# HybridRobotics/ilqr-iterative-tasks

Measured on AMD Instinct MI355X. Metric: batched iLQR iterations/s (n=6,m=2,N=20), higher is better.
Workload: dtype f64

## Files before the change

### ilqr_iterative_tasks_amd/csrc/i2lqr_abi.hip

```cpp
#include <hip/hip_runtime.h>
#include <dlfcn.h>
#include <rccl/rccl.h>

#include <atomic>
#include <cmath>
#include <cstdarg>
#include <cstdio>
#include <cstdlib>
#include <cstring>
#include <mutex>
#include <new>
#include <unordered_set>

#include "../../include/i2lqr.h"
#include "i2lqr_devcfg.hpp"
#include "i2lqr_geometry.hpp"
#include "i2lqr_group.h"
#include "i2lqr_lane.hpp"
#include "i2lqr_select.hpp"
#include "i2lqr_wave.hpp"

#include "i2lqr_lane12.h"

#define I2LQR_DRY_RUN_LANE 1
// ... 203 lines not shown
#ifdef I2LQR_DEBUG
  if (rc != I2LQR_OK) return rc;
  unsigned long long* w = i2lqr::debug_trap_word();
  if (!w) return rc;
  hipStreamCaptureStatus cap = hipStreamCaptureStatusNone;
  if (hipStreamIsCapturing((hipStream_t)stream, &cap) == hipSuccess &&
      cap != hipStreamCaptureStatusNone)
    return rc;
  if (hipStreamSynchronize((hipStream_t)stream) != hipSuccess)
    return fail(I2LQR_ERR_LAUNCH, "debug build: the stream reported an error");
  unsigned long long rec = 0;
  if (hipMemcpy(&rec, w, sizeof(rec), hipMemcpyDeviceToHost) != hipSuccess)
    return fail(I2LQR_ERR_LAUNCH, "debug build: could not read the violation record");
  if (rec) {
    (void)hipMemset(w, 0, sizeof(rec));
    static const char* const names[] = {"?", "wave-kernel LDS slice", "eight-lane LDS slice",
                                        "sixteen-lane LDS slice", "quad12 HBM workspace slot",
                                        "lane kernel row of X", "lane kernel row of U / k",
                                        "lane kernel row of K", "lane kernel LDS word",
                                        "compaction row / problem index"};
    const int tag = (int)((rec >> 56) & 0x7f);
    return fail(I2LQR_ERR_LAUNCH, "debug build: index check failed: %s, index %lld, limit %lld",
                names[tag < 10 ? tag : 0], (long long)((rec >> 28) & 0xfffffff),
                (long long)(rec & 0xfffffff));
  }
#else
  (void)stream;
#endif
  return rc;
}
}

struct i2lqr_handle {
  i2lqr_config cfg;
  int lanes;
  size_t lds_bytes;
  int device;
  void* ws;
  int64_t ws_bytes;
  int64_t compact_min_batch;
  int opt_defer, opt_reroll, opt_lds_steps, opt_merge, opt_ckpt, opt_stagger;
  int wave_tail;
  int opt_pair;
  int opt_two_x;
  int opt_chunk_step;
  int opt_fuse;
  int opt_final_round;
  int opt_first_chunk;
  int opt_fstep;
  int opt_group;
  int opt_spec;
  int opt_group_ws;
  int opt_group_overlap;
  int opt_group_fixed;
  struct Epilogue {
    const int32_t* qfun;
    int outer_iter, max_relax_iter;
    void* cost_it;
    void* part;
    int64_t* best_idx;
    void* best_cost;
    bool fused;
  };
  static constexpr unsigned kTickets = 16;
  unsigned* ticket;
  std::atomic<unsigned> ticket_next;
  hipEvent_t ev_ready, ev_side_done;
  bool side_pending;
  DeviceGeometry geo;
};

namespace {
thread_local i2lqr_handle::Epilogue* t_epi = nullptr;
}

namespace {

enum FusedKernel { K_WAVE, K_GROUP, K_GROUP16, K_GROUP_WS, K_SPEC, K_SPEC16, K_QUAD, K_INVALID };
constexpr int64_t kAutoGroupBatch = 1024;
constexpr int64_t kAutoSpecBatch = 12288;

FusedKernel select_fused(const i2lqr_handle* h, int64_t B, bool early_exit, const char** why) {
  static const char* none = "";
  if (!why) why = &none;
  const bool m2 = h->cfg.m == 2 && h->cfg.n + h->cfg.m <= 8;
  const bool q16 = h->cfg.n + h->cfg.m == 16;
  if (m2) {
    const bool can = group_supported(h->cfg);
    if (h->opt_group == 8 && !can) {
      *why = "\"group_lanes\" = 8 needs a bicycle plant with Q = R = 0 and a horizon whose eight "
             "problem slices fit a CU's LDS";
      return K_INVALID;
    }
    const bool can_spec16 = group_spec_supported(h->cfg, 16), can_spec8 = group_spec_supported(h->cfg, 8);
    const bool spec16 = h->opt_group == 16 || (h->opt_group < 0 && can_spec16);
    const bool can_spec = spec16 ? can_spec16 : can_spec8;
    if (h->opt_spec == 1 && !can_spec) {
      *why = "\"speculate\" = 1 needs the eight- / sixteen-lane kernel and a horizon whose speculative "
             "buffers fit a CU's LDS";
      return K_INVALID;
    }
    if (can_spec && h->opt_group != 64 &&
        (h->opt_spec == 1 ||
         (h->opt_spec < 0 && h->opt_group < 0 && early_exit && B <= h->geo.scaled(kAutoSpecBatch))))
      return spec16 ? K_SPEC16 : K_SPEC;
    const bool can16 = group16_supported(h->cfg);
// ... 84 lines not shown
           {(const void*)k_iterate<T, Sys, LANES, false>, (const void*)k_iterate<T, Sys, LANES, true>,
            (const void*)k_backward<T, Sys, LANES, false>, (const void*)k_backward<T, Sys, LANES, true>,
            (const void*)k_forward<T, Sys, LANES, false>, (const void*)k_forward<T, Sys, LANES, true>,
            (const void*)k_rollout<T, Sys, LANES, false>, (const void*)k_rollout<T, Sys, LANES, true>})
        HIP_TRY(hipFuncSetAttribute(kernel, hipFuncAttributeMaxDynamicSharedMemorySize,
                                    (int)h->lds_bytes));
    return I2LQR_OK;
  }

  static int iterate(i2lqr_handle* h, int64_t B, int n_iters, int early_exit, void* X, void* U,
                     const void* x_term, void* lamb, const void* obs, void* cost, void* K, void* k,
                     int32_t* iters, int32_t* status, hipStream_t s) {
    const Cfg c = make_dev_cfg<T, n, m>(h->cfg);
    IterArgs<T> a = iter_args<T>(B, n_iters, early_exit, X, U, x_term, lamb, obs, cost, K, k, iters,
                                 status);
#ifdef I2LQR_STAMPS
    a.dbg = (unsigned long long*)h->ws;
#endif
    const char* why = "";
    const FusedKernel fk = select_fused(h, B, early_exit != 0, &why);
    if (t_epi && (fk == K_GROUP || fk == K_GROUP16 || fk == K_GROUP_WS)) {
      a.qfun = t_epi->qfun;
      a.outer_iter = t_epi->outer_iter;
      a.max_relax_iter = t_epi->max_relax_iter;
      a.cost_it = (T*)t_epi->cost_it;
      if (t_epi->best_idx) {
        a.pick_part = (MinPair<T>*)t_epi->part;
        a.pick_ticket = h->ticket + h->ticket_next.fetch_add(1, std::memory_order_relaxed) %
                                        i2lqr_handle::kTickets;
        a.best_idx = t_epi->best_idx;
        a.best_cost = (T*)t_epi->best_cost;
      }
      t_epi->fused = true;
    }
    switch (fk) {
      case K_INVALID:
        return fail(I2LQR_ERR_UNSUPPORTED, "%s", why);
      case K_SPEC:
      case K_SPEC16:
        if constexpr (m == 2 && n + m <= 8) {
          HIP_TRY(group_spec_iterate<T>(h->cfg, a, s, fk == K_SPEC16 ? 16 : 8));
          return I2LQR_OK;
        }
        break;
      case K_GROUP:
        if constexpr (m == 2 && n + m <= 8) {
          HIP_TRY(group_iterate<T>(h->cfg, a, s));
          return I2LQR_OK;
        }
        break;
      case K_GROUP16:
        if constexpr (m == 2 && n + m <= 8) {
          HIP_TRY(group16_iterate<T>(h->cfg, a, s, h->opt_group_overlap != 0,
                                     h->opt_group_fixed != 0));
          return I2LQR_OK;
        }
        break;
      case K_GROUP_WS:
        if constexpr (m == 2 && n + m <= 8) {
          HIP_TRY(group_iterate_ws<T>(h->cfg, a, h->ws, s));
          return I2LQR_OK;
        }
        break;
      case K_QUAD:
        if constexpr (n + m == 16) {
          HIP_TRY(quad_iterate<T>(h->cfg, a, h->ws, s));
          return I2LQR_OK;
        }
        break;
      case K_WAVE:
        break;
    }
    const size_t lds_f = fstep_lds_bytes(h->cfg.N);
    const int64_t waves_per_cu = (grid(B) + h->geo.cus - 1) / h->geo.cus;
    const bool fstep = kHasFstep && lds_f <= h->geo.default_dyn_lds &&
                       (h->opt_fstep >= 0 ? h->opt_fstep != 0
                                          : waves_per_cu * lds_f <= h->geo.lds_per_cu - 10 * 1024);
    if constexpr (kHasFstep) {
      if (fstep) {
        with_weights(c.flags, [&](auto W) {
          hipLaunchKernelGGL((k_iterate<T, Sys, LANES, W, true>), dim3(grid(B)), dim3(64), lds_f, s, c, a);
        });
        HIP_TRY(hipGetLastError());
        return I2LQR_OK;
      }
    }
    with_weights(c.flags, [&](auto W) {
      hipLaunchKernelGGL((k_iterate<T, Sys, LANES, W>), dim3(grid(B)), dim3(64), h->lds_bytes, s, c, a);
    });
    HIP_TRY(hipGetLastError());
    return I2LQR_OK;
  }
  static int names_pair(i2lqr_handle*, int64_t, int) { return 0; }
  static int solve_chained(i2lqr_handle* h, int64_t L, int k, void* X, void* U, const void* x_term,
                           void* lamb, const void* obs, void* cost, void* K, void* kk, int32_t* iters,
                           int32_t* status, hipStream_t s) {
    if constexpr (m == 2 && n + m <= 8) {
      if (h->opt_spec == 0 || h->opt_group == 8 || h->opt_group == 64 ||
          !group_spec_chain_supported(h->cfg, L))
        return fail(I2LQR_ERR_UNSUPPORTED, "chains run on the sixteen-lane speculative kernel: a "
                    "bicycle plant with Q = R = 0, at most %lld chains, a horizon whose three-wavefront "
                    "buffers fit a CU's LDS (solve the chain steps one after the other instead)",
                    (long long)h->geo.scaled(512));
      IterArgs<T> a = iter_args<T>(L, h->cfg.max_iter, 1, X, U, x_term, lamb, obs, cost, K, kk, iters,
                                   status);
      a.chain_len = k;
      HIP_TRY(group_spec_chain<T>(h->cfg, a, s));
// ... 753 lines not shown
  }
  if (cfg->n != n || cfg->m != m)
    return fail(I2LQR_ERR_INVALID, "system %d has n=%d m=%d, config says n=%d m=%d", cfg->system_id,
                n, m, cfg->n, cfg->m);
  if (cfg->N < 1 || cfg->N > I2LQR_MAX_HORIZON)
    return fail(I2LQR_ERR_INVALID, "horizon %d outside [1, %d]", cfg->N, I2LQR_MAX_HORIZON);
  if (cfg->dtype != I2LQR_F64 && cfg->dtype != I2LQR_F32)
    return fail(I2LQR_ERR_INVALID, "unknown dtype %d", cfg->dtype);
  if (cfg->layout != I2LQR_LAYOUT_PROBLEM_MAJOR && cfg->layout != I2LQR_LAYOUT_BATCH_MINOR &&
      cfg->layout != I2LQR_LAYOUT_BATCH_TILED)
    return fail(I2LQR_ERR_INVALID, "unknown layout %d", cfg->layout);
  if (!(cfg->dt > 0) || !(cfg->lamb_factor > 1) || cfg->max_iter < 0)
    return fail(I2LQR_ERR_INVALID, "need dt > 0, lamb_factor > 1, max_iter >= 0");
  for (int a = 0; a < m; a++)
    if (!(cfg->u_max[a] > 0)) return fail(I2LQR_ERR_INVALID, "u_max[%d] must be > 0", a);
  if (cfg->layout != I2LQR_LAYOUT_PROBLEM_MAJOR) {
    for (int i = 0; i < n; i++)
      for (int j = 0; j < i; j++)
        if (cfg->Q[i * I2LQR_MAX_N + j] != cfg->Q[j * I2LQR_MAX_N + i] ||
            cfg->Qt[i * I2LQR_MAX_N + j] != cfg->Qt[j * I2LQR_MAX_N + i])
          return fail(I2LQR_ERR_UNSUPPORTED, "the batch-minor / batch-tiled layouts need "
                      "symmetric Q and Qterminal (use the problem-major layout otherwise)");
    for (int a = 0; a < m; a++)
      for (int b = 0; b < a; b++)
        if (cfg->R[a * I2LQR_MAX_M + b] != cfg->R[b * I2LQR_MAX_M + a])
          return fail(I2LQR_ERR_UNSUPPORTED, "the batch-minor / batch-tiled layouts need a "
                      "symmetric R (use the problem-major layout otherwise)");
  }
  int ndev = 0;
#ifdef I2LQR_DRY_RUN
  const bool dry_run = dry::on();
#else
  constexpr bool dry_run = false;
#endif
  if (!dry_run && (hipGetDeviceCount(&ndev) != hipSuccess || ndev <= 0))
    return fail(I2LQR_ERR_NODEVICE, "no HIP device visible (this library has no CPU path)");
  i2lqr_handle* h = new (std::nothrow) i2lqr_handle;
  if (!h) return fail(I2LQR_ERR_LAUNCH, "out of host memory");
  h->cfg = *cfg;
  h->geo = device_geometry();
  if (h->geo.wave != 64) {
    const int w = h->geo.wave;
    delete h;
    return fail(I2LQR_ERR_UNSUPPORTED, "the kernels are built for 64-lane wavefronts (gfx950), this "
                "device reports %d", w);
  }
  h->ws = nullptr;
  h->ws_bytes = 0;
  h->compact_min_batch = -1;
  h->opt_defer = h->opt_reroll = h->opt_lds_steps = h->opt_fstep = h->opt_group = -1;
  h->opt_merge = h->opt_ckpt = h->opt_spec = h->opt_stagger = h->opt_group_ws = -1;
  h->opt_group_overlap = -1;
  h->opt_group_fixed = -1;
  h->wave_tail = -1;
  h->opt_first_chunk = -1;
  h->opt_fuse = -1;
  h->opt_final_round = -1;
  h->opt_chunk_step = -1;
  h->opt_pair = -1;
  h->opt_two_x = -1;
  h->ticket = nullptr;
  h->ticket_next.store(0);
  h->ev_ready = h->ev_side_done = nullptr;
  h->side_pending = false;
  constexpr size_t kTicketBytes = i2lqr_handle::kTickets * sizeof(unsigned);
  if (dry_run) {
#ifdef I2LQR_DRY_RUN
    static unsigned fake_tickets[i2lqr_handle::kTickets];
    h->device = 0;
    h->ticket = fake_tickets;
    dry::allow(fake_tickets, sizeof(fake_tickets));
#endif
  } else if (hipGetDevice(&h->device) != hipSuccess ||
      hipMalloc((void**)&h->ticket, kTicketBytes) != hipSuccess ||
      hipMemset(h->ticket, 0, kTicketBytes) != hipSuccess) {
    if (h->ticket) (void)hipFree(h->ticket);
    delete h;
    return fail(I2LQR_ERR_LAUNCH, "could not set up the handle's device state: %s",
                hipGetErrorString(hipGetLastError()));
  }
  const int rc = dispatch(h, [&](auto L) { return L.prepare(h); });
  if (rc != I2LQR_OK) {
    (void)hipFree(h->ticket);
    delete h;
    return rc;
  }
  {
    std::lock_guard<std::mutex> lock(g_live_mu);
    live_handles().insert(h);
  }
  *out = h;
  g_err[0] = 0;
  return I2LQR_OK;
}

int64_t i2lqr_dry_run(int32_t op, void* p, int64_t n) {
#ifdef I2LQR_DRY_RUN
  switch (op) {
    case 0: return dry::on() ? 1 : 0;
    case 1: if (!dry::on()) break; dry::allow(p, (size_t)n); return 0;
    case 2: if (!dry::on()) break; dry::reset(); return 0;
    case 3: if (!dry::on()) break; return dry::report((char*)p, n);
    default: return fail(I2LQR_ERR_INVALID, "i2lqr_dry_run: unknown operation %d", op);
  }
  return fail(I2LQR_ERR_UNSUPPORTED, "dry-run launches need I2LQR_DRY_RUN=1 in the environment");
#else
// ... 93 lines not shown
  for (int a = 0; a < cfg->m; a++)
    for (int b = 0; b < cfg->m; b++)
      if (cfg->R[a * I2LQR_MAX_M + b] != cfg->R[b * I2LQR_MAX_M + a]) lane_ok = false;
  int64_t from;
  switch (cfg->system_id) {
    case I2LQR_SYS_BICYCLE4:
    case I2LQR_SYS_BICYCLE6:
      from = weights ? kLaneFromWeights
                     : (early_exit ? lane_from(*cfg).solve : lane_from(*cfg).iterate);
      break;
    case I2LQR_SYS_QUAD12: {
      const LaneFrom q = kLaneFromQuad[cfg->N <= 31 ? 0 : 1][cfg->dtype == I2LQR_F64 ? 0 : 1];
      from = weights ? kLaneFromWeights : (early_exit ? q.solve : q.iterate);
      if (cfg->dtype != I2LQR_F64 && weights) lane_ok = false;
      break;
    }
    default: return fail(I2LQR_ERR_INVALID, "unknown system_id %d", cfg->system_id);
  }
  from = device_geometry().scaled_from(from);
  if (!lane_ok || B < from) return I2LQR_LAYOUT_PROBLEM_MAJOR;
  return B % 64 == 0 ? I2LQR_LAYOUT_BATCH_TILED : I2LQR_LAYOUT_BATCH_MINOR;
}

int i2lqr_set_compaction(i2lqr_handle* h, int64_t min_batch) {
  if (!h) return fail(I2LQR_ERR_INVALID, "null handle");
  if (h->cfg.layout == I2LQR_LAYOUT_PROBLEM_MAJOR && min_batch > 0)
    return fail(I2LQR_ERR_UNSUPPORTED, "compaction applies to the batch-minor / batch-tiled layouts");
  h->compact_min_batch = min_batch < 0 ? -1 : min_batch;
  return I2LQR_OK;
}

int i2lqr_set_option(i2lqr_handle* h, const char* name, int64_t value) {
  if (!h || !name) return fail(I2LQR_ERR_INVALID, "null handle or option name");
  if (value < -1 || value > 0x7fffffff) return fail(I2LQR_ERR_INVALID, "option value out of range");
  const int v = (int)value;
  if (!strcmp(name, "defer_states")) h->opt_defer = v < 0 ? -1 : (v != 0);
  else if (!strcmp(name, "reroll_nominal")) h->opt_reroll = v < 0 ? -1 : (v != 0);
  else if (!strcmp(name, "lds_gain_steps")) h->opt_lds_steps = v;
  else if (!strcmp(name, "merge_inputs")) h->opt_merge = v < 0 ? -1 : (v != 0);
  else if (!strcmp(name, "checkpoint_states")) h->opt_ckpt = v < 0 ? -1 : (v != 0);
  else if (!strcmp(name, "stagger")) h->opt_stagger = v;
  else if (!strcmp(name, "per_step_jacobians")) h->opt_fstep = v < 0 ? -1 : (v != 0);
  else if (!strcmp(name, "wave_tail")) h->wave_tail = v < 0 ? -1 : (v > 65536 ? 65536 : v);
  else if (!strcmp(name, "first_chunk")) h->opt_first_chunk = v < 1 ? -1 : (v > 1024 ? 1024 : v);
  else if (!strcmp(name, "helper_wavefront")) h->opt_pair = v < 0 ? -1 : (v != 0);
  else if (!strcmp(name, "state_buffers")) h->opt_two_x = v < 0 ? -1 : (v != 0);
  else if (!strcmp(name, "chunk_step")) h->opt_chunk_step = v < 1 ? -1 : (v > 1024 ? 1024 : v);
  else if (!strcmp(name, "fused_compaction")) h->opt_fuse = v < 0 ? -1 : (v != 0);
  else if (!strcmp(name, "final_round")) h->opt_final_round = v < 0 ? -1 : (v > 20 ? 20 : v);
  else if (!strcmp(name, "speculate")) h->opt_spec = v < 0 ? -1 : (v != 0);
  else if (!strcmp(name, "group_workspace")) h->opt_group_ws = v < 0 ? -1 : (v != 0);
  else if (!strcmp(name, "group_overlap")) h->opt_group_overlap = v < 0 ? -1 : (v != 0);
  else if (!strcmp(name, "group_fixed_horizon")) h->opt_group_fixed = v < 0 ? -1 : (v != 0);
  else if (!strcmp(name, "debug_self_test")) {
#ifdef I2LQR_DEBUG
    unsigned long long* w = i2lqr::debug_trap_word();
    double* buf = nullptr;
    HIP_TRY(hipMalloc((void**)&buf, 8 * sizeof(double)));
    hipLaunchKernelGGL(k_debug_self_test, dim3(1), dim3(64), 0, (hipStream_t)0, buf, w);
    const int rc = debug_check(I2LQR_OK, nullptr);
    (void)hipFree(buf);
    return rc;
#else
    return fail(I2LQR_ERR_UNSUPPORTED, "\"debug_self_test\" exists in the index-checked debug build "
                "only (make -C ilqr_iterative_tasks_amd/csrc debug)");
#endif
  }
  else if (!strcmp(name, "group_lanes")) {
    if (v != -1 && v != 8 && v != 16 && v != 64)
      return fail(I2LQR_ERR_INVALID, "\"group_lanes\" is 8, 16, 64 or -1");
    h->opt_group = v;
  }
  else return fail(I2LQR_ERR_INVALID, "unknown option '%s'", name);
  return I2LQR_OK;
}

static const char* kernel_name(const i2lqr_handle* h, int64_t B, bool early_exit) {
  if (!h) return "";
  if (h->cfg.layout != I2LQR_LAYOUT_PROBLEM_MAJOR) {
    if (h->cfg.system_id == I2LQR_SYS_QUAD12) return "k_lane_iterate_rows";
    const auto pair = [&](auto L) {
      return L.names_pair(const_cast<i2lqr_handle*>(h), B, early_exit ? 1 : 0);
    };
    return dispatch(h, pair) == 1 ? "k_lane_iterate_pair" : "k_lane_iterate";
  }
  switch (select_fused(h, B, early_exit, nullptr)) {
    case K_SPEC: return "k_group_spec";
    case K_SPEC16: return "k_group_spec (sixteen lanes)";
    case K_GROUP: return "k_group_iterate";
    case K_GROUP16: return "k_group_iterate (sixteen lanes)";
    case K_GROUP_WS: return "k_group_iterate (workspace form)";
    case K_QUAD: return "k_quad_iterate";
    case K_WAVE: return "k_iterate";
    default: return "unsupported";
  }
}

const char* i2lqr_iterate_kernel(const i2lqr_handle* h, int64_t B) { return kernel_name(h, B, false); }
const char* i2lqr_solve_kernel(const i2lqr_handle* h, int64_t B) { return kernel_name(h, B, true); }

int i2lqr_set_workspace(i2lqr_handle* h, void* workspace, int64_t bytes) {
  if (!h) return fail(I2LQR_ERR_INVALID, "null handle");
  if (bytes < 0 || (bytes > 0 && !workspace) || ((uintptr_t)workspace & 15))
    return fail(I2LQR_ERR_INVALID, "workspace must be a 16-byte aligned device pointer");
  h->ws = workspace;
  h->ws_bytes = bytes;
// ... 558 lines not shown
```

### ilqr_iterative_tasks_amd/csrc/i2lqr_group.h

```cpp
#pragma once
#include <hip/hip_runtime.h>

#include "../../include/i2lqr.h"
#include "i2lqr_wave.hpp"

namespace i2lqr {

bool group_supported(const i2lqr_config& cfg);
template <class T> hipError_t group_iterate(const i2lqr_config& cfg, const IterArgs<T>& a,
                                            hipStream_t stream);

constexpr int64_t kGroup16Batch = 4096;
bool group16_supported(const i2lqr_config& cfg);
template <class T> hipError_t group16_iterate(const i2lqr_config& cfg, const IterArgs<T>& a,
                                              hipStream_t stream, bool overlap = true,
                                              bool fixed = true);
#define I2LQR_GROUP_FIXED_HORIZONS(X) X(20)
bool group16_fixed_horizon(int N);
template <class T> hipError_t group16_iterate_fixed(const i2lqr_config& cfg, const IterArgs<T>& a,
                                                    hipStream_t stream, int wavefronts);

constexpr int64_t kGroupWsBatch = 4096;
constexpr int64_t kGroupWsTop = 8192;
constexpr int64_t kGroupWsTopF32 = 7168;
inline int64_t group_ws_top(const i2lqr_config& cfg) {
  return cfg.dtype == I2LQR_F64 ? kGroupWsTop : kGroupWsTopF32;
}
int64_t group_workspace_bytes(const i2lqr_config& cfg, int64_t B);
template <class T> hipError_t group_iterate_ws(const i2lqr_config& cfg, const IterArgs<T>& a,
                                               void* ws, hipStream_t stream);

bool group_spec_supported(const i2lqr_config& cfg, int lanes);
template <class T> hipError_t group_spec_iterate(const i2lqr_config& cfg, const IterArgs<T>& a,
                                                 hipStream_t stream, int lanes);
bool group_spec_chain_supported(const i2lqr_config& cfg, int64_t chains);
template <class T> hipError_t group_spec_chain(const i2lqr_config& cfg, const IterArgs<T>& a,
                                               hipStream_t stream);
bool group_spec_tail_supported(const i2lqr_config& cfg);
template <class T> hipError_t group_spec_tail(const i2lqr_config& cfg, const IterArgs<T>& a,
                                              hipStream_t stream);

bool quad_supported(const i2lqr_config& cfg);
int64_t quad_workspace_bytes(const i2lqr_config& cfg, int64_t B);
template <class T> hipError_t quad_iterate(const i2lqr_config& cfg, const IterArgs<T>& a, void* ws,
                                           hipStream_t stream);

}
```

### ilqr_iterative_tasks_amd/csrc/i2lqr_group.hip

```cpp
#include "i2lqr_group.h"

#include "i2lqr_devcfg.hpp"
#include "i2lqr_geometry.hpp"
#include "i2lqr_group.hpp"
#include "i2lqr_dryrun.hpp"
#include "i2lqr_group_launch.hpp"

namespace i2lqr {

namespace {

template <class T, class Sys, int H, int G = kGroup>
hipError_t launch_h(const i2lqr_config& cfg, const IterArgs<T>& a, hipStream_t s) {
  const auto c = make_dev_cfg<T, Sys::n, Sys::m>(cfg);
  const size_t lds = group_lds_bytes<T, Sys, G>(cfg.N);
  if (hipError_t e = raise_lds_limit<k_group_iterate<T, Sys, H, false, G>>(lds); e != hipSuccess)
    return e;
  constexpr int PW = 64 / G;
  const unsigned grid = (unsigned)((a.B + PW - 1) / PW);
  hipLaunchKernelGGL((k_group_iterate<T, Sys, H, false, G>), dim3(grid), dim3(64 * H), lds, s, c, a,
                     (T*)nullptr);
  return hipGetLastError();
}
template <class T, class Sys>
hipError_t launch16(const i2lqr_config& cfg, const IterArgs<T>& a, hipStream_t s, bool overlap,
                    bool fixed) {
  const int64_t cus = device_geometry().cus;
  int wavefronts = 1;
#ifndef I2LQR_STAMPS
  if (overlap && (a.B + 3) / 4 <= cus) wavefronts = 3;
  else if ((a.B + 3) / 4 <= 2 * cus) wavefronts = 2;
  if (fixed && group16_fixed_horizon(cfg.N)) return group16_iterate_fixed<T>(cfg, a, s, wavefronts);
#endif
  if (wavefronts == 3) return launch_h<T, Sys, 3, 16>(cfg, a, s);
  if (wavefronts == 2) return launch_h<T, Sys, 2, 16>(cfg, a, s);
  return launch_h<T, Sys, 1, 16>(cfg, a, s);
}
template <class T, class Sys>
hipError_t launch_ws(const i2lqr_config& cfg, const IterArgs<T>& a, void* ws, hipStream_t s) {
  const auto c = make_dev_cfg<T, Sys::n, Sys::m>(cfg);
  const size_t lds = (size_t)GLayout<Sys>(cfg.N, true).wave_words() * sizeof(T);
  if (hipError_t e = raise_lds_limit<k_group_iterate<T, Sys, 1, true>>(lds); e != hipSuccess) return e;
  const unsigned grid = (unsigned)((a.B + kGroupsPerWave - 1) / kGroupsPerWave);
  hipLaunchKernelGGL((k_group_iterate<T, Sys, 1, true>), dim3(grid), dim3(64), lds, s, c, a, (T*)ws);
  return hipGetLastError();
}

template <class T, class Sys>
hipError_t launch(const i2lqr_config& cfg, const IterArgs<T>& a, hipStream_t s) {
  const int64_t cus = device_geometry().cus;
#ifndef I2LQR_STAMPS
  if ((a.B + kGroupsPerWave - 1) / kGroupsPerWave <= cus) return launch_h<T, Sys, 3>(cfg, a, s);
#endif
  return launch_h<T, Sys, 1>(cfg, a, s);
}

constexpr int kSpecWideBatch = 512;

template <class T, class Sys, int V, int G = kGroup> size_t spec_lds_bytes(int N) {
  return (size_t)GSpecLayout<Sys, V, G>(N).group_words() * sizeof(T);
}

template <class T, class Sys, int V, bool SETIO, int G>
hipError_t launch_spec_v(const i2lqr_config& cfg, const IterArgs<T>& a, hipStream_t s) {
  const auto c = make_dev_cfg<T, Sys::n, Sys::m>(cfg);
  const size_t lds = spec_lds_bytes<T, Sys, V, G>(cfg.N);
  if (hipError_t e = raise_lds_limit<k_group_spec<T, Sys, V, SETIO, G>>(lds); e != hipSuccess)
    return e;
  constexpr int PW = 64 / G;
  const int64_t problems = SETIO ? (int64_t)a.count_max : a.B;
  const unsigned grid = (unsigned)((problems + PW - 1) / PW);
  hipLaunchKernelGGL((k_group_spec<T, Sys, V, SETIO, G>), dim3(grid), dim3(64 * V), lds, s, c, a);
  return hipGetLastError();
}
template <class T, class Sys, bool SETIO, int G>
hipError_t launch_spec(const i2lqr_config& cfg, const IterArgs<T>& a, hipStream_t s) {
  const DeviceGeometry& geo = device_geometry();
  const bool wide = !SETIO && a.B <= geo.scaled(kSpecWideBatch) &&
                    spec_lds_bytes<T, Sys, 3, G>(cfg.N) <= geo.max_dyn_lds;
  if (wide) return launch_spec_v<T, Sys, 3, SETIO, G>(cfg, a, s);
  return launch_spec_v<T, Sys, 2, SETIO, G>(cfg, a, s);
}
template <class T, bool SETIO>
hipError_t launch_spec_any(const i2lqr_config& cfg, const IterArgs<T>& a, hipStream_t s, int lanes) {
  return visit_bicycle<T>(cfg, [&](auto, auto sys) {
    using Sys = decltype(sys);
// ... 19 lines not shown
  });
  return lds <= device_geometry().max_dyn_lds;
}

}

bool group_spec_supported(const i2lqr_config& cfg, int lanes) {
  if (!spec_plant_ok(cfg) || cfg.layout != I2LQR_LAYOUT_PROBLEM_MAJOR) return false;
  return lanes == 16 ? spec_lds_fits<16>(cfg) : (group_supported(cfg) && spec_lds_fits<kGroup>(cfg));
}
int group_spec_tail_lanes(const i2lqr_config& cfg) {
  if (!spec_plant_ok(cfg)) return 0;
  return spec_lds_fits<16>(cfg) ? 16 : (spec_lds_fits<kGroup>(cfg) ? kGroup : 0);
}
bool group_spec_tail_supported(const i2lqr_config& cfg) { return group_spec_tail_lanes(cfg) != 0; }

template <class T, class Sys>
hipError_t launch_spec_chain(const i2lqr_config& cfg, const IterArgs<T>& a, hipStream_t s) {
  const auto c = make_dev_cfg<T, Sys::n, Sys::m>(cfg);
  const size_t lds = spec_lds_bytes<T, Sys, 3, 16>(cfg.N);
  if (hipError_t e = raise_lds_limit<k_group_spec<T, Sys, 3, false, 16, true>>(lds); e != hipSuccess)
    return e;
  const unsigned grid = (unsigned)((a.B + 3) / 4);
  hipLaunchKernelGGL((k_group_spec<T, Sys, 3, false, 16, true>), dim3(grid), dim3(64 * 3), lds, s, c, a);
  return hipGetLastError();
}
bool group_spec_chain_supported(const i2lqr_config& cfg, int64_t chains) {
  if (!spec_plant_ok(cfg) || cfg.layout != I2LQR_LAYOUT_PROBLEM_MAJOR) return false;
  const DeviceGeometry& geo = device_geometry();
  if (chains > geo.scaled(kSpecWideBatch)) return false;
  const size_t lds = visit_bicycle(cfg, [&](auto t, auto sys) {
    return spec_lds_bytes<decltype(t), decltype(sys), 3, 16>(cfg.N);
  });
  return lds <= geo.max_dyn_lds;
}
template <class T>
hipError_t group_spec_chain(const i2lqr_config& cfg, const IterArgs<T>& a, hipStream_t s) {
  return visit_bicycle<T>(cfg, [&](auto, auto sys) {
    return launch_spec_chain<T, decltype(sys)>(cfg, a, s);
  });
}
template <class T>
hipError_t group_spec_iterate(const i2lqr_config& cfg, const IterArgs<T>& a, hipStream_t s, int lanes) {
  return launch_spec_any<T, false>(cfg, a, s, lanes);
}
template <class T>
hipError_t group_spec_tail(const i2lqr_config& cfg, const IterArgs<T>& a, hipStream_t s) {
  return launch_spec_any<T, true>(cfg, a, s, group_spec_tail_lanes(cfg));
}

bool group16_supported(const i2lqr_config& cfg) { return group_lds_fits<16>(cfg); }
template <class T>
hipError_t group16_iterate(const i2lqr_config& cfg, const IterArgs<T>& a, hipStream_t s, bool overlap,
                           bool fixed) {
  return visit_bicycle<T>(cfg, [&](auto, auto sys) {
    return launch16<T, decltype(sys)>(cfg, a, s, overlap, fixed);
  });
}

bool group_supported(const i2lqr_config& cfg) { return group_lds_fits<kGroup>(cfg); }

int64_t group_workspace_bytes(const i2lqr_config& cfg, int64_t B) {
  if (!group_supported(cfg) || B <= 0) return 0;
  const int64_t probs = (B + kGroupsPerWave - 1) / kGroupsPerWave * kGroupsPerWave;
  const int64_t words = visit_bicycle<double>(cfg, [&](auto, auto sys) {
    return GLayout<decltype(sys)>(cfg.N, true).ws_words();
  });
  const size_t lds = visit_bicycle(cfg, [&](auto t, auto sys) {
    return (size_t)GLayout<decltype(sys)>(cfg.N, true).wave_words() * sizeof(t);
  });
  if (lds > device_geometry().max_dyn_lds) return 0;
  return probs * words * (cfg.dtype == I2LQR_F64 ? 8 : 4);
}
template <class T>
hipError_t group_iterate_ws(const i2lqr_config& cfg, const IterArgs<T>& a, void* ws, hipStream_t s) {
  return visit_bicycle<T>(cfg, [&](auto, auto sys) {
    return launch_ws<T, decltype(sys)>(cfg, a, ws, s);
  });
}

template <class T>
hipError_t group_iterate(const i2lqr_config& cfg, const IterArgs<T>& a, hipStream_t s) {
  return visit_bicycle<T>(cfg, [&](auto, auto sys) { return launch<T, decltype(sys)>(cfg, a, s); });
}

#define I2LQR_GROUP_LAUNCHERS(T)                                                                    \
  template hipError_t group_iterate<T>(const i2lqr_config&, const IterArgs<T>&, hipStream_t);       \
  template hipError_t group16_iterate<T>(const i2lqr_config&, const IterArgs<T>&, hipStream_t, bool, \
                                         bool);                                                    \
  template hipError_t group_iterate_ws<T>(const i2lqr_config&, const IterArgs<T>&, void*,           \
                                          hipStream_t);                                             \
  template hipError_t group_spec_iterate<T>(const i2lqr_config&, const IterArgs<T>&, hipStream_t,   \
                                            int);                                                   \
  template hipError_t group_spec_chain<T>(const i2lqr_config&, const IterArgs<T>&, hipStream_t);    \
  template hipError_t group_spec_tail<T>(const i2lqr_config&, const IterArgs<T>&, hipStream_t);
I2LQR_GROUP_LAUNCHERS(double)
I2LQR_GROUP_LAUNCHERS(float)

}
```

### ilqr_iterative_tasks_amd/csrc/i2lqr_group.hpp

```cpp
#pragma once
#include <hip/hip_runtime.h>
#include <stdint.h>

#include "i2lqr_systems.hpp"
#include "i2lqr_wave.hpp"

namespace i2lqr {

constexpr int kGroup = 8;
constexpr int kGroupsPerWave = 64 / kGroup;

template <class Sys> struct GroupPattern {
  static constexpr int n = Sys::n, m = Sys::m, W = n + m, NV = Sys::NVAR;
  static constexpr int dt_row(int b) {
    for (int i = 2; i < n; i++)
      if (i != b && Sys::pat(i, b) == 2) return i;
    return -1;
  }
  static constexpr bool column_ok(int b) {
    int extra = 0;
    for (int i = 0; i < n; i++) {
      const int code = Sys::pat(i, b);
      if (i < 2) {
        if (code == 2) return false;
// ... 252 lines not shown
    const T spd_y = opt == 1 ? ob[4] : T(0), spd_x = opt == 2 ? ob[4] : T(0);
    const int rounds = (N + stride) / stride;
    for (int r = 0; r < rounds; r++) {
      const int t0 = first + r * stride;
      const int t = t0 < N ? t0 : N;
      const int ts = t0 < N ? t0 : N - 1;
      T* Rs = rec(ts);
      {
        T xe[n], tr[NT], u[m], jv[NV];
#pragma unroll
        for (int i = 0; i < n; i++) xe[i] = S[XUo + (ts + 1) * W + i];
#pragma unroll
        for (int a = 0; a < m; a++) u[a] = S[XUo + ts * W + n + a];
#pragma unroll
        for (int q = 0; q < NT; q++) tr[q] = S[TRo + (ts + 1) * NT + q];
        Sys::jac_var(c, xe, u, tr, jv);
#pragma unroll
        for (int q = 0; q < NV; q++) Rs[GL::R_JV + q] = jv[q];
#pragma unroll
        for (int a = 0; a < m; a++) {
          T e_hi, e_lo;
          if (sizeof(T) == 8 && c.fast_barrier) {
            e_hi = t_exp_bounded(c.ctrl_q2 * (u[a] - c.u_max[a]));
            e_lo = c.ctrl_c[a] * t_rcp(e_hi);
          } else {
            e_hi = t_exp(c.ctrl_q2 * (u[a] - c.u_max[a]));
            e_lo = t_exp(c.ctrl_q2 * (-c.u_max[a] - u[a]));
          }
          Rs[GL::R_LU + a] = c.ctrl_q12 * e_hi - c.ctrl_q12 * e_lo;
          Rs[GL::R_LUU + a] = c.ctrl_q122 * e_hi +
                              c.ctrl_q122 * e_lo;
        }
      }
      T* R = rec(t);
      R[GL::R_ZERO] = T(0);
      R[GL::R_ONE] = T(1);
      const T px = S[XUo + t * W + 0], py = S[XUo + t * W + 1];
      const T dz = opt == 2 ? px - (ob[0] - T(t) * spd_x) : px - ob[0];
      const T dy = opt == 1 ? py - (ob[1] + T(t) * spd_y) : py - ob[1];
      const T h = T(1) + c.safety_margin - (dz * pa * dz + dy * pb * dy);
      const T hd0 = T(-2) * pa * dz, hd1 = T(-2) * pb * dy;
      const T e = t_exp(c.obs_q2 * h);
      const T c1 = c.obs_q12 * e, c2 = c.obs_q122 * e;
      R[GL::R_OB + 0] = has_ob ? c1 * hd0 : T(0);
      R[GL::R_OB + 1] = has_ob ? c1 * hd1 : T(0);
      R[GL::R_OB + 2] = has_ob ? c2 * (hd0 * hd0) : T(0);
      R[GL::R_OB + 3] = has_ob ? c2 * (hd0 * hd1) : T(0);
      R[GL::R_OB + 4] = has_ob ? c2 * (hd1 * hd1) : T(0);
    }
    wave_sync();
    ws_publish();
  }

  __device__ __forceinline__ void quu_inverse(const T (&Quu)[m * m], T lamb, T (&inv)[m * m]) const {
    static_assert(m == 2, "the eight-lane kernel is written for m == 2 plants");
    t_quu_inverse2(Quu, lamb, inv);
  }

  template <bool GENERAL>
  __device__ __forceinline__ bool backward(int XUo, const T (&xT)[n], T lamb, bool commit) const {
    if constexpr (G == 16) return backward_row<GENERAL>(XUo, xT, lamb, commit);
    bool bad = false;
    T va[n];
    {
      const T* Rn = rec(N);
      T dx[n];
#pragma unroll
      for (int i = 0; i < n; i++) dx[i] = S[XUo + N * W + i] - xT[i];
#pragma unroll
      for (int i = 0; i < n; i++) {
        T vxx = T(0), vx = T(0);
#pragma unroll
        for (int r = 0; r < n; r++) {
          const T q = T(2) * Qt[i * n + r];
          vxx = (g == r) ? q : vxx;
          vx += q * dx[r];
        }
        va[i] = (g == n) ? vx : vxx;
      }
      va[0] += Rn[off_l0];
      va[1] += Rn[off_l1];
    }
    const int gcol = g < GL::KW ? g : GL::KW - 1;
    struct Rec { T jv[NV], luu[m], c0, c1, l0, l1, lrow[m]; };
    Rec ra, rb;
    auto load_record = [&](int t, Rec& r) __attribute__((always_inline)) {
      const T* R = rec(t);
#pragma unroll
      for (int q = 0; q < NV; q++) r.jv[q] = R[GL::R_JV + q];
#pragma unroll
      for (int a = 0; a < m; a++) r.luu[a] = R[GL::R_LUU + a];
      r.c0 = R[off_c0];
      r.c1 = R[off_c1];
      r.l0 = R[off_l0];
      r.l1 = R[off_l1];
#pragma unroll
      for (int a = 0; a < m; a++) r.lrow[a] = R[off_lu[a]];
    };
    load_record(N - 1, ra);
    auto step = [&](const int t, Rec& rc, Rec& rn) __attribute__((always_inline)) {
      if constexpr (WS) load_record(t > 0 ? t - 1 : 0, rn);
      const T (&jv)[NV] = rc.jv;
      const T (&luu)[m] = rc.luu;
      const T (&lrow)[m] = rc.lrow;
      const T c0 = rc.c0, c1 = rc.c1, l0 = rc.l0, l1 = rc.l1;
      STAMP_BEGIN();
// ... 85 lines not shown
#pragma unroll
      for (int a = 0; a < m; a++) {
        T acc = T(0);
#pragma unroll
        for (int b = 0; b < m; b++) acc = t_fma(Quu[a * m + b], kc[b], acc);
        qk[a] = acc;
      }
#pragma unroll
      for (int i = 0; i < n; i++) {
        T acc = T(0);
#pragma unroll
        for (int a = 0; a < m; a++) acc = t_fma(kr[a][i], qk[a], acc);
        va[i] = h[i] - acc;
      }
      STAMP_END(5);
    };
    int t = N - 1;
    if constexpr (I2LQR_GROUP_UNROLL >= 4) {
      for (; t >= 3; t -= 4) {
        step(t, ra, rb);
        step(t - 1, rb, ra);
        step(t - 2, ra, rb);
        step(t - 3, rb, ra);
      }
    }
    for (; t >= 1; t -= 2) {
      step(t, ra, rb);
      step(t - 1, rb, ra);
    }
    if (t == 0) step(0, ra, rb);
    ws_publish();
    return bad;
  }

  template <bool GENERAL>
  __device__ __forceinline__ bool backward_row(int XUo, const T (&xT)[n], T lamb, bool commit) const {
    T vb[n];
    terminal_base(XUo, xT, vb);
    return backward_row_from<GENERAL>(vb, lamb, commit);
  }
  __device__ __forceinline__ void terminal_base(int XUo, const T (&xT)[n], T (&vb)[n]) const {
    T dx[n];
#pragma unroll
    for (int i = 0; i < n; i++) dx[i] = S[XUo + N * W + i] - xT[i];
    const int gq = g < n ? g : 0;
#pragma unroll
    for (int i = 0; i < n; i++) {
      T vx = T(0);
#pragma unroll
      for (int r = 0; r < n; r++) vx += (T(2) * Qt[i * n + r]) * dx[r];
      const T vxx = T(2) * Qt[i * n + gq];
      vb[i] = (g == n) ? vx : (g < n ? vxx : T(0));
    }
  }
  template <bool GENERAL>
  __device__ __forceinline__ bool backward_row_from(const T (&vb)[n], T lamb, bool commit) const {
    static_assert(GL::KW > n + 1, "the padding word of a gain row takes the stores of idle lanes");
    bool bad = false;
    T va[n];
    {
      const T* Rn = rec(N);
#pragma unroll
      for (int i = 0; i < n; i++) va[i] = vb[i];
      va[0] += Rn[off_l0];
      va[1] += Rn[off_l1];
    }
    const int gcol = (commit && g <= n) ? g : GL::KW - 1;
    T cdr[n];
#pragma unroll
    for (int r = 0; r < n; r++) cdr[r] = (rsrc == r) ? cdt : T(0);
    struct Rec { T jv[NV], luu[m], c0, c1, l0, l1, lrow[m]; };
    Rec ra, rb;
    constexpr bool FIXED = NH > 0 && !GENERAL;
    const T* const R0 = rec(0);
    const T *pc0 = R0, *pc1 = R0, *pl0 = R0, *pl1 = R0, *plu[m];
#pragma unroll
    for (int a = 0; a < m; a++) plu[a] = R0;
    if constexpr (FIXED) {
      pc0 = R0 + off_c0; pc1 = R0 + off_c1; pl0 = R0 + off_l0; pl1 = R0 + off_l1;
#pragma unroll
      for (int a = 0; a < m; a++) plu[a] = R0 + off_lu[a];
    }
    auto load_record = [&](int t, Rec& r) __attribute__((always_inline)) {
      if constexpr (FIXED) {
        const int o = t * GL::RW;
#pragma unroll
        for (int q = 0; q < NV; q++) r.jv[q] = R0[o + GL::R_JV + q];
#pragma unroll
        for (int a = 0; a < m; a++) r.luu[a] = R0[o + GL::R_LUU + a];
        r.c0 = pc0[o];
        r.c1 = pc1[o];
        r.l0 = pl0[o];
        r.l1 = pl1[o];
#pragma unroll
        for (int a = 0; a < m; a++) r.lrow[a] = plu[a][o];
      } else {
        const T* R = rec(t);
#pragma unroll
        for (int q = 0; q < NV; q++) r.jv[q] = R[GL::R_JV + q];
#pragma unroll
        for (int a = 0; a < m; a++) r.luu[a] = R[GL::R_LUU + a];
        r.c0 = R[off_c0];
        r.c1 = R[off_c1];
        r.l0 = R[off_l0];
        r.l1 = R[off_l1];
#pragma unroll
// ... 264 lines not shown
      for (int i = 0; i < n; i++) S[XUn + (t + 1) * W + i] = xn[i];
#pragma unroll
      for (int i = 0; i < n; i++) x[i] = xn[i];
    };
    int t = 0;
    if constexpr (WS) {
      for (; t + 1 < N; t += 2) {
        step(t, ga, gb);
        step(t + 1, gb, ga);
      }
      if (t < N) step(t, ga, gb);
    } else {
      if constexpr (I2LQR_GROUP_UNROLL >= 4) {
        for (; t + 3 < N; t += 4) {
          step(t, ga, ga);
          step(t + 1, ga, ga);
          step(t + 2, ga, ga);
          step(t + 3, ga, ga);
        }
      }
      for (; t + 1 < N; t += 2) {
        step(t, ga, ga);
        step(t + 1, ga, ga);
      }
      if (t < N) step(t, ga, ga);
    }
    Sys::template trig_g<GENERAL>(x, tr, bad);
#pragma unroll
    for (int q = 0; q < NT; q++) S[TRn + N * NT + q] = tr[q];
    const T cost = terminal_cost(x, xT);
    wave_sync();
    return cost;
  }
};

__device__ __forceinline__ int idx_div(int e, int d, float rcp_d) {
  int q = (int)((float)e * rcp_d);
  const int r = e - q * d;
  q += (r >= d) ? 1 : 0;
  q -= (r < 0) ? 1 : 0;
  return q;
}

template <class T, class Sys, int H, bool WS, int G, int NH>
__device__ __forceinline__ void group_iterate_body(const DevCfg<T, Sys::n, Sys::m>& c,
                                                   const IterArgs<T>& a, T* ws) {
  static_assert(!(WS && H > 1), "the workspace form runs without helper wavefronts");
  constexpr int n = Sys::n, m = Sys::m, W = n + m;
#ifdef I2LQR_STAMPS
  constexpr bool OVL = false;
#else
  constexpr bool OVL = G == 16 && H >= 3;
#endif
  using GL = GLayout<Sys, G>;
  extern __shared__ __align__(16) unsigned char gsmem_raw[];
  T* smem = reinterpret_cast<T*>(gsmem_raw);
  const int lane = threadIdx.x & 63, hv = threadIdx.x >> 6;
#ifdef I2LQR_STAMPS
  unsigned long long st_k0, st_k1, st_k2, st_k3;
  asm volatile("s_memtime %0\n\ts_waitcnt lgkmcnt(0)" : "=s"(st_k0)::"memory");
#endif
  const int64_t prob0 = (int64_t)blockIdx.x * GL::PW + lane / G;
  const bool real = prob0 < a.B;
  const int64_t prob = real ? prob0 : a.B - 1;
  GroupWorker<T, Sys, WS, G, NH> w(c, smem, lane);
  const int N = NH > 0 ? NH : c.N, g = w.g;
  const float rN = 1.0f / (float)N, rN1 = 1.0f / (float)(N + 1), rnN = 1.0f / (float)(n * N);
  const GL& L = w.L;
  const auto S = w.S;
  if constexpr (WS) w.Wp = ws + prob0 * (int64_t)L.ws_words();

  if (H == 1 || hv == 0) {
    const T* gX = a.X + prob * (int64_t)(n * (N + 1));
    if (g < n) S[L.XU0 + g] = gX[g * (N + 1)];
    const T* gU = a.U + prob * (int64_t)(m * N);
    for (int e = g; e < m * N; e += G) {
      const int aa = idx_div(e, N, rN), t = e - aa * N;
      S[L.XU0 + t * W + n + aa] = gU[e];
    }
    for (int e = lane; e < n * n; e += 64) smem[L.qt_base() + e] = c.Qt[e];
  }
  T xT[n], ob[6];
#pragma unroll
  for (int i = 0; i < n; i++) xT[i] = a.x_term[prob * n + i];
#pragma unroll
  for (int q = 0; q < 6; q++) ob[q] = a.obs ? a.obs[prob * 6 + q] : T(q == 5 ? -1 : 1);
  T lamb = a.lamb[prob];
  wave_sync();

  int cur = 0;
  const T ob_pa = T(1) / (ob[2] * ob[2]), ob_pb = T(1) / (ob[3] * ob[3]);
  int* const ctl = reinterpret_cast<int*>(smem + L.ctl_base());
  if constexpr (H > 1) {
    if (hv > 0) {
      const int h0 = OVL ? hv - 1 : hv, hs = OVL ? H - 1 : H;
      for (;;) {
        __syncthreads();
        const int flags = ctl[8];
        if (!(flags & 1)) break;
        if (flags & 2) {
          const int pc = ctl[lane / G];
          w.prep(pc ? L.XU1 : L.XU0, pc ? L.TR1 : L.TR0, ob, ob_pa, ob_pb, h0 * G + g, hs * G);
        }
        __syncthreads();
      }
      if constexpr (OVL) {
        if (real && a.K) {
          T* const gK = a.K + prob * (int64_t)(m * n * N);
          T* const gk = a.k + prob * (int64_t)(m * N);
          for (int t = h0 * G + g; t < N; t += hs * G) {
            const T* Kt = w.gain(t);
            T kv[m][n + 1];
#pragma unroll
            for (int aa = 0; aa < m; aa++)
#pragma unroll
              for (int j = 0; j <= n; j++) kv[aa][j] = Kt[aa * GL::KW + j];
#pragma unroll
            for (int aa = 0; aa < m; aa++) {
#pragma unroll
              for (int j = 0; j < n; j++) gK[(aa * n + j) * N + t] = kv[aa][j];
              gk[aa * N + t] = kv[aa][n];
            }
          }
        }
      }
      return;
    }
  }
  T vb[n];
#pragma unroll
  for (int i = 0; i < n; i++) vb[i] = T(0);
  T cost = w.rollout(L.XU0, L.TR0, xT);
  int it = 0, status = a.early_exit ? 2  : 0 ;
  T cost_ret = cost;
  bool fresh = true, active = a.n_iters > 0;
#ifdef I2LQR_STAMPS
  asm volatile("s_memtime %0\n\ts_waitcnt lgkmcnt(0)" : "=s"(st_k1)::"memory");
#endif
  while (__any(active)) {
    const int XUo = cur ? L.XU1 : L.XU0, XUn = cur ? L.XU0 : L.XU1;
    const int TRo = cur ? L.TR1 : L.TR0, TRn = cur ? L.TR0 : L.TR1;
#ifdef I2LQR_STAMPS
    {
      auto& st_t0 = w.st_t0; auto& st_t1 = w.st_t1; auto& st_acc = w.st_acc;
      STAMP_BEGIN();
      if (__any(fresh)) w.prep(XUo, TRo, ob, ob_pa, ob_pb, g, G);
      STAMP_END(0);
    }
#else
    if constexpr (H > 1) {
      const bool do_prep = __any(fresh);
      if (g == 0) ctl[lane / G] = cur;
      if (lane == 0) ctl[8] = 1 | (do_prep ? 2 : 0);
      __syncthreads();
      if constexpr (OVL) {
        if (do_prep) w.terminal_base(XUo, xT, vb);
      } else {
        if (do_prep) w.prep(XUo, TRo, ob, ob_pa, ob_pb, g, H * G);
      }
      __syncthreads();
    } else {
      if (__any(fresh)) w.prep(XUo, TRo, ob, ob_pa, ob_pb, g, G);
    }
#endif
    if constexpr (OVL) {
      if (__builtin_expect(__any(w.template backward_row_from<false>(vb, lamb, active)), 0))
        w.template backward_row_from<true>(vb, lamb, active);
    } else {
      if (__builtin_expect(__any(w.template backward<false>(XUo, xT, lamb, active)), 0))
        w.template backward<true>(XUo, xT, lamb, active);
    }
    T cost_new;
    {
#ifdef I2LQR_STAMPS
      auto& st_t0 = w.st_t0; auto& st_t1 = w.st_t1; auto& st_acc = w.st_acc;
      STAMP_BEGIN();
#endif
      bool big = false;
      cost_new = w.template forward<false>(XUo, XUn, TRn, xT, &big);
      if (__builtin_expect(__any(big), 0)) cost_new = w.template forward<true>(XUo, XUn, TRn, xT, &big);
#ifdef I2LQR_STAMPS
      STAMP_END(6);
#endif
    }
    {
      const bool acc = active && cost_new < cost, rej = active && !(cost_new < cost);
      const T lamb_dn = lamb / c.lamb_factor, lamb_up = lamb * c.lamb_factor;
      const bool conv = t_abs((cost_new - cost) / cost) < c.eps;
      it += active ? 1 : 0;
      fresh = acc;
      cur ^= acc ? 1 : 0;
      lamb = acc ? lamb_dn : (rej ? lamb_up : lamb);
      cost_ret = acc ? cost_new : (rej ? cost : cost_ret);
      cost = acc ? cost_new : cost;
      const bool stop_conv = acc && conv, stop_lamb = rej && lamb > c.max_lamb;
      const int ended = stop_conv ? 1 : 3;
      if (a.early_exit) {
        status = (stop_conv || stop_lamb) ? ended : status;
        active = active && !(stop_conv || stop_lamb);
      } else {
        status = (status == 0 && (stop_conv || stop_lamb)) ? ended : status;
      }
      active = active && it < a.n_iters;
    }
  }
#ifdef I2LQR_STAMPS
  asm volatile("s_memtime %0\n\ts_waitcnt lgkmcnt(0)" : "=s"(st_k2)::"memory");
#endif
  if constexpr (H > 1) {
// ... 335 lines not shown
```

### ilqr_iterative_tasks_amd/csrc/i2lqr_group_fixed.hip

```cpp
#include "i2lqr_group.h"

#include "i2lqr_devcfg.hpp"
#include "i2lqr_group.hpp"
#include "i2lqr_dryrun.hpp"
#include "i2lqr_group_launch.hpp"

namespace i2lqr {

namespace {

template <class T, class Sys, int H, int NH>
hipError_t launch_fixed_h(const i2lqr_config& cfg, const IterArgs<T>& a, hipStream_t s) {
  const auto c = make_dev_cfg<T, Sys::n, Sys::m>(cfg);
  const size_t lds = group_lds_bytes<T, Sys, 16>(cfg.N);
  if (hipError_t e = raise_lds_limit<k_group_iterate_fixed<T, Sys, H, NH>>(lds); e != hipSuccess)
    return e;
  const unsigned grid = (unsigned)((a.B + 3) / 4);
  hipLaunchKernelGGL((k_group_iterate_fixed<T, Sys, H, NH>), dim3(grid), dim3(64 * H), lds, s, c, a);
  return hipGetLastError();
}
template <class T, class Sys, int NH>
hipError_t launch_fixed(const i2lqr_config& cfg, const IterArgs<T>& a, hipStream_t s, int helpers) {
  if (helpers == 3) return launch_fixed_h<T, Sys, 3, NH>(cfg, a, s);
  if (helpers == 2) return launch_fixed_h<T, Sys, 2, NH>(cfg, a, s);
  return launch_fixed_h<T, Sys, 1, NH>(cfg, a, s);
}

}

bool group16_fixed_horizon(int N) {
#define I2LQR_X(NH) if (N == NH) return true;
  I2LQR_GROUP_FIXED_HORIZONS(I2LQR_X)
#undef I2LQR_X
  return false;
}

template <class T>
hipError_t group16_iterate_fixed(const i2lqr_config& cfg, const IterArgs<T>& a, hipStream_t s,
                                 int wavefronts) {
  return visit_bicycle<T>(cfg, [&](auto, auto sys) -> hipError_t {
    using Sys = decltype(sys);
#define I2LQR_X(NH) if (cfg.N == NH) return launch_fixed<T, Sys, NH>(cfg, a, s, wavefronts);
    I2LQR_GROUP_FIXED_HORIZONS(I2LQR_X)
#undef I2LQR_X
    return hipErrorInvalidValue;
  });
}

template hipError_t group16_iterate_fixed<double>(const i2lqr_config&, const IterArgs<double>&,
                                                  hipStream_t, int);
template hipError_t group16_iterate_fixed<float>(const i2lqr_config&, const IterArgs<float>&,
                                                 hipStream_t, int);

}
```

Before: 82.00 million.

## Split per-step record prep across six helper wavefronts by record part

When the overlapped group16 kernel applies (batch small enough for one block per CU), the block now launches 7 wavefronts instead of 3. The six helper wavefronts divide the per-step record preparation by part: one part covers the Jacobian and obstacle terms, and each of the m control-barrier terms gets its own part. The main wavefront's terminal value setup now uses DPP row broadcasts. The aim is to shorten the prep phase that the backward pass overlaps with, at the cost of more wavefronts per block, more barrier participants and possible occupancy or register pressure. It can be disabled with the new group_record_parts option.

Result: no change. 82.42 million, median of 6 (+0.5%).

```diff
diff --git a/ilqr_iterative_tasks_amd/csrc/i2lqr_abi.hip b/ilqr_iterative_tasks_amd/csrc/i2lqr_abi.hip
--- a/ilqr_iterative_tasks_amd/csrc/i2lqr_abi.hip
+++ b/ilqr_iterative_tasks_amd/csrc/i2lqr_abi.hip
@@ -279,6 +279,7 @@
   int opt_spec;
   int opt_group_ws;
   int opt_group_overlap;
+  int opt_group_parts;
   int opt_group_fixed;
   struct Epilogue {
     const int32_t* qfun;
@@ -469,7 +470,7 @@
       case K_GROUP16:
         if constexpr (m == 2 && n + m <= 8) {
           HIP_TRY(group16_iterate<T>(h->cfg, a, s, h->opt_group_overlap != 0,
-                                     h->opt_group_fixed != 0));
+                                     h->opt_group_fixed != 0, h->opt_group_parts != 0));
           return I2LQR_OK;
         }
         break;
@@ -1329,6 +1330,7 @@
   h->opt_merge = h->opt_ckpt = h->opt_spec = h->opt_stagger = h->opt_group_ws = -1;
   h->opt_group_overlap = -1;
   h->opt_group_fixed = -1;
+  h->opt_group_parts = -1;
   h->wave_tail = -1;
   h->opt_first_chunk = -1;
   h->opt_fuse = -1;
@@ -1528,6 +1530,11 @@
   else if (!strcmp(name, "group_workspace")) h->opt_group_ws = v < 0 ? -1 : (v != 0);
   else if (!strcmp(name, "group_overlap")) h->opt_group_overlap = v < 0 ? -1 : (v != 0);
   else if (!strcmp(name, "group_fixed_horizon")) h->opt_group_fixed = v < 0 ? -1 : (v != 0);
+  else if (!strcmp(name, "group_record_parts")) {
+    if (v != -1 && v != 0)
+      return fail(I2LQR_ERR_INVALID, "\"group_record_parts\" is 0 or -1");
+    h->opt_group_parts = v;
+  }
   else if (!strcmp(name, "debug_self_test")) {
 #ifdef I2LQR_DEBUG
     unsigned long long* w = i2lqr::debug_trap_word();
diff --git a/ilqr_iterative_tasks_amd/csrc/i2lqr_group.h b/ilqr_iterative_tasks_amd/csrc/i2lqr_group.h
--- a/ilqr_iterative_tasks_amd/csrc/i2lqr_group.h
+++ b/ilqr_iterative_tasks_amd/csrc/i2lqr_group.h
@@ -12,9 +12,10 @@
 
 constexpr int64_t kGroup16Batch = 4096;
 bool group16_supported(const i2lqr_config& cfg);
+constexpr int kGroup16SplitWavefronts = 7;
 template <class T> hipError_t group16_iterate(const i2lqr_config& cfg, const IterArgs<T>& a,
                                               hipStream_t stream, bool overlap = true,
-                                              bool fixed = true);
+                                              bool fixed = true, bool split_records = true);
 #define I2LQR_GROUP_FIXED_HORIZONS(X) X(20)
 bool group16_fixed_horizon(int N);
 template <class T> hipError_t group16_iterate_fixed(const i2lqr_config& cfg, const IterArgs<T>& a,
diff --git a/ilqr_iterative_tasks_amd/csrc/i2lqr_group.hip b/ilqr_iterative_tasks_amd/csrc/i2lqr_group.hip
--- a/ilqr_iterative_tasks_amd/csrc/i2lqr_group.hip
+++ b/ilqr_iterative_tasks_amd/csrc/i2lqr_group.hip
@@ -24,14 +24,16 @@
 }
 template <class T, class Sys>
 hipError_t launch16(const i2lqr_config& cfg, const IterArgs<T>& a, hipStream_t s, bool overlap,
-                    bool fixed) {
+                    bool fixed, bool split_records) {
   const int64_t cus = device_geometry().cus;
   int wavefronts = 1;
 #ifndef I2LQR_STAMPS
-  if (overlap && (a.B + 3) / 4 <= cus) wavefronts = 3;
+  if (overlap && (a.B + 3) / 4 <= cus) wavefronts = split_records ? kGroup16SplitWavefronts : 3;
   else if ((a.B + 3) / 4 <= 2 * cus) wavefronts = 2;
   if (fixed && group16_fixed_horizon(cfg.N)) return group16_iterate_fixed<T>(cfg, a, s, wavefronts);
 #endif
+  if (wavefronts == kGroup16SplitWavefronts)
+    return launch_h<T, Sys, kGroup16SplitWavefronts, 16>(cfg, a, s);
   if (wavefronts == 3) return launch_h<T, Sys, 3, 16>(cfg, a, s);
   if (wavefronts == 2) return launch_h<T, Sys, 2, 16>(cfg, a, s);
   return launch_h<T, Sys, 1, 16>(cfg, a, s);
@@ -157,9 +159,9 @@
 bool group16_supported(const i2lqr_config& cfg) { return group_lds_fits<16>(cfg); }
 template <class T>
 hipError_t group16_iterate(const i2lqr_config& cfg, const IterArgs<T>& a, hipStream_t s, bool overlap,
-                           bool fixed) {
-  return visit_bicycle<T>(cfg, [&](auto, auto sys) {
-    return launch16<T, decltype(sys)>(cfg, a, s, overlap, fixed);
+                           bool fixed, bool split_records) {
+  return visit_bicycle<T>(cfg, [&](auto, auto sys) {
+    return launch16<T, decltype(sys)>(cfg, a, s, overlap, fixed, split_records);
   });
 }
 
@@ -192,7 +194,7 @@
 #define I2LQR_GROUP_LAUNCHERS(T)                                                                    \
   template hipError_t group_iterate<T>(const i2lqr_config&, const IterArgs<T>&, hipStream_t);       \
   template hipError_t group16_iterate<T>(const i2lqr_config&, const IterArgs<T>&, hipStream_t, bool, \
-                                         bool);                                                    \
+                                         bool, bool);                                              \
   template hipError_t group_iterate_ws<T>(const i2lqr_config&, const IterArgs<T>&, void*,           \
                                           hipStream_t);                                             \
   template hipError_t group_spec_iterate<T>(const i2lqr_config&, const IterArgs<T>&, hipStream_t,   \
diff --git a/ilqr_iterative_tasks_amd/csrc/i2lqr_group.hpp b/ilqr_iterative_tasks_amd/csrc/i2lqr_group.hpp
--- a/ilqr_iterative_tasks_amd/csrc/i2lqr_group.hpp
+++ b/ilqr_iterative_tasks_amd/csrc/i2lqr_group.hpp
@@ -328,6 +328,73 @@
     ws_publish();
   }
 
+  static constexpr int kRecordParts = m + 1;
+  __device__ __forceinline__ void prep_parts(int XUo, int TRo, const T (&ob)[6], T pa, T pb, int part,
+                                             int first, int stride) const {
+    static_assert(!WS, "parts of a record in the LDS slice");
+    const bool do_jac = part == 0, do_obs = part == 0;
+    bool do_in[m];
+#pragma unroll
+    for (int a = 0; a < m; a++) do_in[a] = part == 1 + a;
+    const bool has_ob = ob[5] >= T(0);
+    const int opt = has_ob ? (int)ob[5] : 0;
+    const T spd_y = opt == 1 ? ob[4] : T(0), spd_x = opt == 2 ? ob[4] : T(0);
+    const int rounds = (N + stride) / stride;
+    for (int r = 0; r < rounds; r++) {
+      const int t0 = first + r * stride;
+      const int t = t0 < N ? t0 : N;
+      const int ts = t0 < N ? t0 : N - 1;
+      T* Rs = rec(ts);
+      if (do_jac) {
+        T xe[n], tr[NT], u[m], jv[NV];
+#pragma unroll
+        for (int i = 0; i < n; i++) xe[i] = S[XUo + (ts + 1) * W + i];
+#pragma unroll
+        for (int a = 0; a < m; a++) u[a] = S[XUo + ts * W + n + a];
+#pragma unroll
+        for (int q = 0; q < NT; q++) tr[q] = S[TRo + (ts + 1) * NT + q];
+        Sys::jac_var(c, xe, u, tr, jv);
+#pragma unroll
+        for (int q = 0; q < NV; q++) Rs[GL::R_JV + q] = jv[q];
+      }
+      static_for_i<0, m>([&](auto a_) {
+        constexpr int a = decltype(a_)::value;
+        if (do_in[a]) {
+          const T ua = S[XUo + ts * W + n + a];
+          T e_hi, e_lo;
+          if (sizeof(T) == 8 && c.fast_barrier) {
+            e_hi = t_exp_bounded(c.ctrl_q2 * (ua - c.u_max[a]));
+            e_lo = c.ctrl_c[a] * t_rcp(e_hi);
+          } else {
+            e_hi = t_exp(c.ctrl_q2 * (ua - c.u_max[a]));
+            e_lo = t_exp(c.ctrl_q2 * (-c.u_max[a] - ua));
+          }
+          Rs[GL::R_LU + a] = c.ctrl_q12 * e_hi - c.ctrl_q12 * e_lo;
+          Rs[GL::R_LUU + a] = c.ctrl_q122 * e_hi +
+                              c.ctrl_q122 * e_lo;
+        }
+      });
+      if (do_obs) {
+        T* R = rec(t);
+        R[GL::R_ZERO] = T(0);
+        R[GL::R_ONE] = T(1);
+        const T px = S[XUo + t * W + 0], py = S[XUo + t * W + 1];
+        const T dz = opt == 2 ? px - (ob[0] - T(t) * spd_x) : px - ob[0];
+        const T dy = opt == 1 ? py - (ob[1] + T(t) * spd_y) : py - ob[1];
+        const T h = T(1) + c.safety_margin - (dz * pa * dz + dy * pb * dy);
+        const T hd0 = T(-2) * pa * dz, hd1 = T(-2) * pb * dy;
+        const T e = t_exp(c.obs_q2 * h);
+        const T c1 = c.obs_q12 * e, c2 = c.obs_q122 * e;
+        R[GL::R_OB + 0] = has_ob ? c1 * hd0 : T(0);
+        R[GL::R_OB + 1] = has_ob ? c1 * hd1 : T(0);
+        R[GL::R_OB + 2] = has_ob ? c2 * (hd0 * hd0) : T(0);
+        R[GL::R_OB + 3] = has_ob ? c2 * (hd0 * hd1) : T(0);
+        R[GL::R_OB + 4] = has_ob ? c2 * (hd1 * hd1) : T(0);
+      }
+    }
+    wave_sync();
+  }
+
   __device__ __forceinline__ void quu_inverse(const T (&Quu)[m * m], T lamb, T (&inv)[m * m]) const {
     static_assert(m == 2, "the eight-lane kernel is written for m == 2 plants");
     t_quu_inverse2(Quu, lamb, inv);
@@ -519,6 +586,22 @@
       const T vxx = T(2) * Qt[i * n + gq];
       vb[i] = (g == n) ? vx : (g < n ? vxx : T(0));
     }
+  }
+  __device__ __forceinline__ void terminal_base_rows(int XUo, const T (&xT)[n], T (&vb)[n]) const {
+    static_assert(G == 16 && n + 1 <= 16, "one problem per 16-lane DPP row");
+    T dx[n];
+#pragma unroll
+    for (int i = 0; i < n; i++) dx[i] = S[XUo + N * W + i] - xT[i];
+    const int gq = g < n ? g : 0;
+    T vx = T(0);
+#pragma unroll
+    for (int r = 0; r < n; r++) vx += (T(2) * Qt[gq * n + r]) * dx[r];
+    static_for_i<0, n>([&](auto i_) {
+      constexpr int i = decltype(i_)::value;
+      const T vxi = bcast_mov<i>(vx);
+      const T vxx = T(2) * Qt[i * n + gq];
+      vb[i] = (g == n) ? vxi : (g < n ? vxx : T(0));
+    });
   }
   template <bool GENERAL>
   __device__ __forceinline__ bool backward_row_from(const T (&vb)[n], T lamb, bool commit) const {
@@ -889,6 +972,8 @@
 #else
   constexpr bool OVL = G == 16 && H >= 3;
 #endif
+  constexpr int P = (OVL && H == 7) ? GroupWorker<T, Sys, WS, G, NH>::kRecordParts : 1;
+  static_assert(P == 1 || (H - 1) % P == 0, "whole helper wavefronts for each part");
   using GL = GLayout<Sys, G>;
   extern __shared__ __align__(16) unsigned char gsmem_raw[];
   T* smem = reinterpret_cast<T*>(gsmem_raw);
@@ -937,7 +1022,13 @@
         if (!(flags & 1)) break;
         if (flags & 2) {
           const int pc = ctl[lane / G];
-          w.prep(pc ? L.XU1 : L.XU0, pc ? L.TR1 : L.TR0, ob, ob_pa, ob_pb, h0 * G + g, hs * G);
+          if constexpr (P > 1) {
+            constexpr int LP = (H - 1) * G / P;
+            const int q = h0 * G + g;
+            w.prep_parts(pc ? L.XU1 : L.XU0, pc ? L.TR1 : L.TR0, ob, ob_pa, ob_pb, q / LP, q % LP, LP);
+          } else {
+            w.prep(pc ? L.XU1 : L.XU0, pc ? L.TR1 : L.TR0, ob, ob_pa, ob_pb, h0 * G + g, hs * G);
+          }
         }
         __syncthreads();
       }
@@ -991,7 +1082,11 @@
       if (lane == 0) ctl[8] = 1 | (do_prep ? 2 : 0);
       __syncthreads();
       if constexpr (OVL) {
-        if (do_prep) w.terminal_base(XUo, xT, vb);
+        if constexpr (P > 1) {
+          if (do_prep) w.terminal_base_rows(XUo, xT, vb);
+        } else {
+          if (do_prep) w.terminal_base(XUo, xT, vb);
+        }
       } else {
         if (do_prep) w.prep(XUo, TRo, ob, ob_pa, ob_pb, g, H * G);
       }
diff --git a/ilqr_iterative_tasks_amd/csrc/i2lqr_group_fixed.hip b/ilqr_iterative_tasks_amd/csrc/i2lqr_group_fixed.hip
--- a/ilqr_iterative_tasks_amd/csrc/i2lqr_group_fixed.hip
+++ b/ilqr_iterative_tasks_amd/csrc/i2lqr_group_fixed.hip
@@ -21,6 +21,8 @@
 }
 template <class T, class Sys, int NH>
 hipError_t launch_fixed(const i2lqr_config& cfg, const IterArgs<T>& a, hipStream_t s, int helpers) {
+  if (helpers == kGroup16SplitWavefronts)
+    return launch_fixed_h<T, Sys, kGroup16SplitWavefronts, NH>(cfg, a, s);
   if (helpers == 3) return launch_fixed_h<T, Sys, 3, NH>(cfg, a, s);
   if (helpers == 2) return launch_fixed_h<T, Sys, 2, NH>(cfg, a, s);
   return launch_fixed_h<T, Sys, 1, NH>(cfg, a, s);
```
